# ssydasheng/GPflow-Slim

Hardware: AMD Instinct MI355X
Metric: GPR log-marginal-likelihood evals/sec + predict_f latency, fp64, N=32768 D=8 (higher is better)
Workload: dtype f64; 1 GPU; RBF(ARD) GPR log-marginal-likelihood, N=32768 D=8 R=1 fp64, X resident in HBM; n=32768, d=8, n_new=1024, parallelism=1 GPU (fused single-GPU path)

## Files before the change

### gpflow-slim_amd/csrc/blocked.hpp

```cpp
#pragma once
#include <cstdint>

#ifndef GPS_TILE
#define GPS_TILE 128
#endif

struct GemmBatch { int64_t batch = 1; int64_t a_rs = 0, a_cs = 0, a_cm = 0, b_rs = 0, b_cs = 0, b_cm = 0, c_rs = 0, c_cs = 0, c_cm = 0; };

template <class Ops>
struct Blocked {
  Ops& ops;
  explicit Blocked(Ops& o) : ops(o) {}
  typedef int64_t i64;

  static i64 split(i64 n) { return ((n / GPS_TILE) / 2) * GPS_TILE; }
  static i64 split_solve(i64 n) {
    const i64 P = 4 * GPS_TILE;
    if (n <= P) return split(n);
    const i64 h = ((n / P) / 2) * P;
    return h > P ? h : P;
  }

  struct Deferred { double* B; i64 ldb, dm, dn; bool issued; };

// ... 220 lines not shown
  int lauum_rec(const double* Y, i64 ldy, i64 n, double* Kv, i64 ldk) {
    if (n <= 0) return 0;
    if (n == GPS_TILE) return ops.gemm(1, 1, n, n, n, Y, ldy, Y, ldy, Kv, ldk);
    const i64 n1 = split(n), n2 = n - n1;
    int rc = lauum_rec(Y, ldy, n1, Kv, ldk);
    if (rc) return rc;
    const double* Y12 = Y + n1;
    const double* Y22 = Y + n1 * ldy + n1;
    rc = ops.gemm(2, 1, n1, n1, n2, Y12, ldy, Y12, ldy, Kv, ldk);
    if (rc) return rc;
    rc = ops.gemm(1,  2, n2, n1, n2, Y22, ldy, Y12, ldy, Kv + n1 * ldk, ldk);
    if (rc) return rc;
    return lauum_rec(Y22, ldy, n2, Kv + n1 * ldk + n1, ldk);
  }

  int trsv_rec(const double* L, i64 ldl, i64 n, i64 blk0, double* y, i64 ldy, i64 r) {
    if (n <= 0 || r <= 0) return 0;
    if (n == GPS_TILE) return ops.trsv_base(blk0, y, ldy, r, L, ldl);
    const i64 n1 = split(n), n2 = n - n1;
    int rc = trsv_rec(L, ldl, n1, blk0, y, ldy, r);
    if (rc) return rc;
    rc = ops.gemv_sub(L + n1 * ldl, ldl, n2, n1, y, y + n1, ldy, r);
    if (rc) return rc;
    return trsv_rec(L + n1 * ldl + n1, ldl, n2, blk0 + n1 / GPS_TILE, y + n1, ldy, r);
  }

  int wide_inverse(const double* L, i64 ldl, i64 nf, i64 wb, const double* linv, const double* linvT, double* W, double* Wt, double* Tm) {
    if (nf <= 0) return 0;
    const i64 T = GPS_TILE, ldt = wb / 2;
    int rc = ops.blocks_to_diag(linv, W, nf / T, wb);
// ... 28 lines not shown
```

### gpflow-slim_amd/csrc/gemm_f64.hip

```cpp
#include "gps_common.hpp"

typedef double v4d __attribute__((ext_vector_type(4)));
typedef double v2d __attribute__((ext_vector_type(2)));

#define BK_MIN 16
#ifndef STRIP
#define STRIP 8
#endif

struct GemmArgs {
  const double* A; const double* B; double* C;
  i64 lda, ldb, ldc;
  int Tm, Tn;
  int K;
  int ntiles;
  int triA;
  int batch, tpb;
  int pair;
  i64 a_rs, a_cs, b_rs, b_cs, c_rs, c_cs, a_cm, b_cm, c_cm;
  int cb_tiles;
  i64 cb_stride;
  int cb_cpack = 0;
  int nfull, nsplit;
  double* ws;
// ... 164 lines not shown
  }
  const i64 nbatch = (bt && bt->batch > 1) ? bt->batch : 1;
  const bool half_rows = (M % 128 == 64) && !lower && triA != 1 && triA != 2 && nbatch == 1;
  if ((M % 128 && !half_rows) || N % 128 || K % BK_MIN || (lower && M < N))
    return gps_fail(h, GPS_ERR_ARG, "gemm_nt: M,N must be multiples of 128 and K of 16 (lower: M >= N)");
  if ((lda & 1) || (ldb & 1) || ((uintptr_t)A & 15) || ((uintptr_t)B & 15))
    return gps_fail(h, GPS_ERR_ARG, "gemm_nt: operands must be 16-byte aligned with even leading dimension");
  const bool rowpanel = (C == A);
  if (rowpanel && (N != 128 || lower || triA || nbatch > 1))
    return gps_fail(h, GPS_ERR_ARG, "gemm_nt: in-place form needs N == 128 (no batch, no triangular operand)");
  GemmArgs g;
  g.A = A; g.B = B; g.C = C; g.lda = lda; g.ldb = ldb; g.ldc = ldc; g.K = (int)K; g.triA = triA;
  g.batch = (int)nbatch; g.tpb = 0;
  g.a_rs = g.a_cs = g.b_rs = g.b_cs = g.c_rs = g.c_cs = g.a_cm = g.b_cm = g.c_cm = 0;
  if (nbatch > 1) {
    if (lower) return gps_fail(h, GPS_ERR_ARG, "gemm_nt: no batched lower-triangle form");
    g.a_rs = bt->a_rs; g.a_cs = bt->a_cs; g.a_cm = bt->a_cm; g.b_rs = bt->b_rs; g.b_cs = bt->b_cs; g.b_cm = bt->b_cm;
    g.c_rs = bt->c_rs; g.c_cs = bt->c_cs; g.c_cm = bt->c_cm;
    if ((g.a_cs & 1) || (g.b_cs & 1) || (g.a_cm & 1) || (g.b_cm & 1)) return gps_fail(h, GPS_ERR_ARG, "gemm_nt: batch column steps must be even");
  }
  g.stamps = h->gemm_stamps;
  g.sig_ptr = h->next_sig_ptr; g.sig_val = h->next_sig_val; h->next_sig_ptr = nullptr;
  g.cb_tiles = 0; g.cb_stride = 0;
  const double t128 = (double)nbatch * (lower ? 0.5 * (double)(N / 128) * (double)(N / 128 + 1) + (double)((M - N) / 128) * (double)(N / 128)
                                             : ((double)M / 128.0) * (double)(N / 128));
  const double flops = triA == 3 ? (double)nbatch * 128.0 * 128.0 * ((double)M / 128.0) * (double)(N / 128) * (double)(N + 128)
                     : triA      ? (double)nbatch * 128.0 * 128.0 * (double)(N / 128) * (double)(M / 128) * (double)(M + 128)
                                 : 2.0 * t128 * 128.0 * 128.0 * (double)K;
  const double bytes = t128 * (((op == 0 || op == 2) ? 2.0 : 1.0) * 128.0 * 128.0 * 8.0) +
                       8.0 * (double)K * (double)(M + N);
  LaunchScope ls(h, KC_GEMM, flops, bytes);
// ... 10 lines not shown
    if (bm == 64) return launch_cfg<64, 128, 2>(h, op, 0, g, M, N);
    if (bm == 32) return launch_cfg<32, 128, 1>(h, op, 0, g, M, N);
    return launch_cfg<16, 128, 1>(h, op, 0, g, M, N);
  }
  int tb = 32;
  if (force) tb = force < 32 ? 32 : force;
  else if (t128 >= target && !half_rows) tb = 128;
  else if (4.0 * t128 >= target) tb = 64;
  if (half_rows && tb > 64) tb = 64;
  if (tb == 128) return launch_cfg<128, 128, 2>(h, op, lower, g, M, N);
  if (tb == 64) return launch_cfg<64, 64, 2>(h, op, lower, g, M, N);
  return launch_cfg<32, 32, 2>(h, op, lower, g, M, N);
}

int gps_launch_gemm_nt_dual(gps_handle_t h, i64 M, i64 N, i64 K, const double* A, i64 lda, const double* B, i64 ldb,
                            double* C, i64 ldc, double* C2, i64 ldc2, int op2) {
  if (M <= 0 || N <= 0 || K <= 0) return GPS_OK;
  if (M % 128 || N % 128 || K % BK_MIN || !C || !C2 || (op2 != 0 && op2 != 2))
    return gps_fail(h, GPS_ERR_ARG, "gemm_nt_dual: M,N must be multiples of 128 and K of 16, two targets, op2 0 or 2");
  if ((lda & 1) || (ldb & 1) || ((uintptr_t)A & 15) || ((uintptr_t)B & 15))
    return gps_fail(h, GPS_ERR_ARG, "gemm_nt_dual: operands must be 16-byte aligned with even leading dimension");
  if (C == A || C2 == A || C == C2) return gps_fail(h, GPS_ERR_ARG, "gemm_nt_dual: no in-place form");
  if ((M / 128) * (N / 128) > 0x7fffffff) return gps_fail(h, GPS_ERR_ARG, "gemm_nt: too many tiles");
  GemmArgs g;
  g.A = A; g.B = B; g.C = C; g.lda = lda; g.ldb = ldb; g.ldc = ldc; g.K = (int)K; g.triA = 0;
  g.batch = 1; g.pair = 0;
  g.a_rs = g.a_cs = g.b_rs = g.b_cs = g.c_rs = g.c_cs = g.a_cm = g.b_cm = g.c_cm = 0;
  g.cb_tiles = 0; g.cb_stride = 0;
  g.Tm = (int)(M / 128); g.Tn = (int)(N / 128);
  g.ntiles = g.Tm * g.Tn; g.tpb = g.ntiles;
  g.nfull = g.ntiles; g.nsplit = 1; g.ws = nullptr; g.cnt = nullptr;
  g.stamps = nullptr;
  g.sig_ptr = h->next_sig_ptr; g.sig_val = h->next_sig_val; h->next_sig_ptr = nullptr;
  g.C2 = C2; g.ldc2 = ldc2; g.op2 = op2;
  const double t128 = (double)g.ntiles;
  LaunchScope ls(h, KC_GEMM, 2.0 * t128 * 128.0 * 128.0 * (double)K, t128 * 4.0 * 128.0 * 128.0 * 8.0 + 8.0 * (double)K * (double)(M + N));
  ls.tag[0] = M; ls.tag[1] = N; ls.tag[2] = K; ls.tag[3] = 50 + op2;
  const size_t lds = (size_t)(2 * (128 + 128) * (16 + 2)) * sizeof(double);
  int rc = gps_dyn_lds(h, reinterpret_cast<const void*>(&gemm_nt_f64_kernel<128, 128, 2, false, 0, 2, 16, true>), (int)lds);
  if (rc) return rc;
  hipLaunchKernelGGL((gemm_nt_f64_kernel<128, 128, 2, false, 0, 2, 16, true>), dim3(g.ntiles), dim3(256), lds, h->stream, g);
  GPS_HIP(h, hipGetLastError());
  return GPS_OK;
}

int gps_launch_gemm_nt_cyclic(gps_handle_t h, i64 M, i64 nblocks, i64 nb, i64 stride, i64 K, const double* A, i64 lda,
                              double* C, i64 ldc, int c_packed) {
  if (M <= 0 || nblocks <= 0) return GPS_OK;
  if (M % 128 || nb % 128 || stride % 128 || K % BK_MIN || stride < nb || (nblocks - 1) * stride + nb > M)
    return gps_fail(h, GPS_ERR_ARG, "gemm_nt_cyclic: sizes must be multiples of 128 and the blocks must lie inside the panel");
  GemmArgs g;
  g.A = A; g.B = A; g.C = C; g.lda = lda; g.ldb = lda; g.ldc = ldc; g.K = (int)K; g.triA = 0;
  g.batch = 1; g.tpb = 0; g.pair = 0; g.a_rs = g.a_cs = g.b_rs = g.b_cs = g.c_rs = g.c_cs = g.a_cm = g.b_cm = g.c_cm = 0;
// ... 15 lines not shown
```

### gpflow-slim_amd/csrc/gps_common.hpp

```cpp
#pragma once
#include <hip/hip_runtime.h>
#include <cmath>
#include <cstdint>
#include <cstdio>
#include <cstring>
#include <cstdlib>
#include <string>
#include <vector>
#include "../../include/gpflowslim_hip.h"
#include "blocked.hpp"

#define GPS_TILE 128
#define GPS_WB 2048
#define GPS_WIDE_MAX_ROWS 8192

typedef int64_t i64;

static inline i64 gps_pad(i64 n) { return ((n + GPS_TILE - 1) / GPS_TILE) * GPS_TILE; }

struct DevBuf;
typedef std::vector<DevBuf*> DevBufList;
struct DevBuf {
  enum Class { WORK, PERSISTENT };
  void*  p = nullptr;
// ... 194 lines not shown
    int on = 1;
    int fault_inject = 0;
    long long fallbacks = 0;
    int consec = 0;
    int cooldown = 0;
    bool defer = false;
    bool pending = false;
    bool valid = false;
    double slog = 0.0, ssq = 0.0;
    bool linvT_stale = false;
  } small;
  DevBuf dGemmWs{bufs}, dGemmCnt{bufs};
  int gemm_strassen_min = 2048;
  static constexpr int strassen_min_builtin = 2048, strassen_lower_min_builtin = 4096;
  int gemm_strassen_lower_min = strassen_lower_min_builtin;
  DevBuf dStrS{bufs}, dStrT{bufs};
  int gemm_strassen_presum_min = 1024;
  double gemm_strassen_presum_max_bytes = 0.0;
  long long strassen_presum_fallbacks = 0;
  DevBuf dStrS5{bufs}, dStrT5{bufs};
  struct RffFactor { bool have = false; unsigned long long gen = 0; i64 F = 0, r = 0; int kind = -1, d = 0; bool refine = false; } rff;
  DevBuf dGemvWs{bufs}, dGemvCnt{bufs};
  struct KgprSolve { bool have = false; unsigned long long gen = 0; i64 m = 0, n = 0; } kgpr;
  int kron_cg_check_every = 8;
  int psi_sum_chunk = 0;
  DevBuf dPsiParts{bufs};
  DevBuf dPsiWork{bufs};
  struct GpmcState { bool have = false; unsigned long long gen = 0; i64 n = 0, k = 0; } gpmc;
};

// ... 98 lines not shown
  GPS_HIP(h, hipFuncSetAttribute(fn, hipFuncAttributeMaxDynamicSharedMemorySize, bytes));
  h->dyn_lds_done.push_back(fn);
  return GPS_OK;
}

int gps_launch_gemm_nt(gps_handle_t h, int op, int lower, i64 M, i64 N, i64 K,
                       const double* A, i64 lda, const double* B, i64 ldb,
                       double* C, i64 ldc);
struct GemmBatch;
int gps_launch_gemm_nt_ex(gps_handle_t h, int op, int lower, int tri, i64 M, i64 N, i64 K,
                          const double* A, i64 lda, const double* B, i64 ldb,
                          double* C, i64 ldc, const GemmBatch* bt);
int gps_launch_gemm_nt_cyclic(gps_handle_t h, i64 M, i64 nblocks, i64 nb, i64 stride, i64 K, const double* A, i64 lda,
                              double* C, i64 ldc, int c_packed = 0);
int gps_launch_gemm_nt_dual(gps_handle_t h, i64 M, i64 N, i64 K, const double* A, i64 lda, const double* B, i64 ldb,
                            double* C, i64 ldc, double* C2, i64 ldc2, int op2);
int gps_launch_block_sum(gps_handle_t h, double* D, i64 ldd, const double* X, i64 ldx, const double* Y, i64 ldy, i64 rows, i64 cols,
                         int sign);
int gps_launch_strassen_sums(gps_handle_t h, int side, const double* X, i64 ldx, i64 rows, i64 cols, double* out, i64 ostride);
int gps_launch_potrf_base(gps_handle_t h, double* A, i64 lda, double* Linv_blk,
                          double* LinvT_blk, int* d_info, i64 row0, int factor,
                          long long* d_stamps = nullptr);
int gps_launch_trsm_leaf_refine(gps_handle_t h, double* B, i64 ldb, i64 m, const double* W, const double* D, i64 ldd,
                                int upper);
int gps_launch_trsv_leaf_refine(gps_handle_t h, const double* Wt, const double* D, i64 ldd, double* y, i64 ldy, i64 r,
                                int upper);
static inline bool gps_gpr_needs_refine(const gps_handle_s* h, double noise_var, double kdiag, i64 n) {
  if (h->leaf_refine >= 0) return h->leaf_refine > 0;
  return !((double)n * kdiag + noise_var <= h->leaf_refine_cond * noise_var);
}

// ... 206 lines not shown
```

### gpflow-slim_amd/csrc/gps_gpr.hip

```cpp
#include "gps_ops.hpp"

static int gpr_lml_finish(gps_handle_t h, i64 r, double* lml);
extern "C" int gps_kmat(gps_handle_t h, const gps_kern_node_t* prog, int n_nodes, const double* X,
                        int64_t n, const double* X2, int64_t m, int64_t d_all, double diag_add,
                        double* K_out) {
  if (!h || !X || !K_out || n < 0 || d_all <= 0) return gps_fail(h, GPS_ERR_ARG, "gps_kmat: bad argument");
  GPS_HIP(h, hipSetDevice(h->device));
  const bool sym = (X2 == nullptr);
  if (sym) m = n;
  if (n == 0 || m == 0) return GPS_OK;
  const i64 prow = ((n + 63) / 64) * 64;
  const i64 pcol = sym ? prow : ((m + 63) / 64) * 64;
  GPS_HIP(h, h->dXnew.ensure((size_t)n * d_all * 8));
  GPS_HIP(h, hipMemcpyAsync(h->dXnew.p, X, (size_t)n * d_all * 8, hipMemcpyHostToDevice, h->stream));
  const double* dX2 = nullptr;
  if (!sym) {
    GPS_HIP(h, h->dTmp3.ensure((size_t)m * d_all * 8));
    GPS_HIP(h, hipMemcpyAsync(h->dTmp3.p, X2, (size_t)m * d_all * 8, hipMemcpyHostToDevice, h->stream));
    dX2 = h->dTmp3.d();
  }
  GPS_HIP(h, h->dTmp.ensure((size_t)prow * pcol * 8));
  int rc = gps_launch_kmat(h, prog, n_nodes, h->dXnew.d(), n, dX2, m, d_all, diag_add, h->dTmp.d(), pcol,
                           prow, pcol,  0,  0);
  if (rc) return rc;
// ... 321 lines not shown
static int gpr_kinv_small(gps_handle_t h, i64 r, double* d_abort, double* d_AT) {
  int rc = gpr_kinv_buffers(h, r);
  if (rc) return rc;
  return gps_launch_small_inverse(h, h->dK.d(), h->npad, h->dLinv.d(), h->dAlpha.d(), r, h->dY.d(), h->dKinv.d(), h->dA.d(), d_abort, d_AT, h->n);
}
static int gpr_kinv_blocked(gps_handle_t h, i64 r) {
  const i64 np = h->npad;
  int rc = gpr_kinv_buffers(h, r);
  if (!rc) rc = gpr_ensure_linvT(h);
  if (rc) return rc;
  HipOps ops = factor_ops(h, h->dLinv.d(), np, (int*)h->dInfo.p);
  Blocked<HipOps> bl(ops);
  GPS_HIP(h, hipMemcpyAsync(h->dA.p, h->dAlpha.p, (size_t)r * np * 8, hipMemcpyDeviceToDevice, h->stream));
  rc = trsv_backward(h, ops, h->dK.d(), np, np, h->dA.d(), np, r);
  if (rc) return rc;
  rc = bl.inv_t_rec(h->dK.d(), np, np, 0, h->dY.d(), np);
  if (rc) return rc;
  return bl.lauum_rec(h->dY.d(), np, np, h->dKinv.d(), np);
}
static int gpr_grad_readback(gps_handle_t h, const gps_kern_node_t* prog, int n_nodes, i64 r, double* grad_slots, double* grad_noise,
                             double* kinv_resid) {
  const i64 n = h->n, np = h->npad;
  int rc = gps_launch_grad(h, prog, n_nodes, h->dX.d(), n, h->d_all, np, h->dKinv.d(), np, h->dA.d(), np, r, nullptr, grad_slots, grad_noise);
  if (rc || !kinv_resid) return rc;
  GPS_HIP(h, h->dTmp2.ensure((size_t)n * r * 8));
  rc = gps_launch_transpose(h, h->dA.d(), np, r, n, h->dTmp2.d(), r);
  if (rc) return rc;
  GPS_HIP(h, hipMemcpyAsync(kinv_resid, h->dTmp2.p, (size_t)n * r * 8, hipMemcpyDeviceToHost, h->stream));
  return GPS_OK;
}
// ... 185 lines not shown
```

### gpflow-slim_amd/csrc/gps_handle.hip

```cpp
#include "gps_ops.hpp"

extern "C" int gps_create(int device_id, gps_handle_t* out) {
  if (!out) return GPS_ERR_ARG;
  *out = nullptr;
  int count = 0;
  if (hipGetDeviceCount(&count) != hipSuccess || count <= 0) return GPS_ERR_HIP;
  if (device_id < 0 || device_id >= count) return GPS_ERR_ARG;
  gps_handle_t h = new gps_handle_s();
  h->device = device_id;
  if (hipSetDevice(device_id) != hipSuccess || hipGetDeviceProperties(&h->prop, device_id) != hipSuccess) {
    delete h;
    return GPS_ERR_HIP;
  }
  if (hipStreamCreateWithFlags(&h->stream, hipStreamNonBlocking) != hipSuccess) { delete h; return GPS_ERR_HIP; }
  for (int i = 0; i < 8; ++i) {
    if (hipEventCreate(&h->ev[i]) != hipSuccess) { delete h; return GPS_ERR_HIP; }
  }
  if (const char* v = getenv("GPS_GEMM_PAIR")) h->gemm_pair = atoi(v);
  if (const char* la = getenv("GPS_LOOKAHEAD")) h->potrf_lookahead = atoi(la);
  if (h->dInfo.ensure(64) != hipSuccess || h->dScal.ensure(4096) != hipSuccess) { delete h; return GPS_ERR_HIP; }
  *out = h;
  return GPS_OK;
}

// ... 98 lines not shown
  }
  return gps_fail(h, GPS_ERR_ARG, "unknown kernel class");
}
extern "C" int gps_last_stage_ms(gps_handle_t h, double* out5) {
  if (!h || !out5) return GPS_ERR_ARG;
  for (int i = 0; i < 5; ++i) out5[i] = h->stage_ms[i];
  return GPS_OK;
}

static int set_strassen_tuning(gps_handle_t h, const char* sub, double value) {
  const bool lower_min = strcmp(sub, "lower_min") == 0;
  if (lower_min || strcmp(sub, "presum_min") == 0) {
    if (value < 0 || value > 1e9 || value != (double)((i64)value) || (i64)value % 128)
      return gps_fail(h, GPS_ERR_ARG, std::string("gemm_strassen_") + sub + ": 0 or a multiple of 128");
    (lower_min ? h->gemm_strassen_lower_min : h->gemm_strassen_presum_min) = (int)value;
    return GPS_OK;
  }
  if (strcmp(sub, "presum_max_bytes") == 0) {
    if (!(value >= 0)) return gps_fail(h, GPS_ERR_ARG, "gemm_strassen_presum_max_bytes: 0 (no cap) or a number of bytes");
    h->gemm_strassen_presum_max_bytes = value;
    return GPS_OK;
  }
  return gps_fail(h, GPS_ERR_ARG, "unknown option");
}

extern "C" int gps_set_option(gps_handle_t h, const char* key, double value) {
  if (!h || !key) return GPS_ERR_ARG;
  if (strcmp(key, "gemm_force_tile") == 0) { h->gemm_force_tb = (int)value; return GPS_OK; }
  if (strcmp(key, "gemm_tail_split") == 0) { h->gemm_tail_split = (int)value; return GPS_OK; }
  if (strcmp(key, "gemm_strassen_min") == 0) {
// ... 37 lines not shown
  return gps_run_mfma_diag(h, waves_per_simd, tflops, layout_ok);
}

extern "C" int gps_diag_gemm_nt(gps_handle_t h, int op, int lower, int64_t m, int64_t n, int64_t k,
                                const double* A, const double* B, double* C) {
  if (!h || !A || !B || !C) return GPS_ERR_ARG;
  GPS_HIP(h, hipSetDevice(h->device));
  const size_t ab = (size_t)m * k * 8, bb = (size_t)n * k * 8, cb = (size_t)m * n * 8;
  GPS_HIP(h, h->dTmp.ensure(ab)); GPS_HIP(h, h->dTmp2.ensure(bb)); GPS_HIP(h, h->dTmp3.ensure(cb));
  GPS_HIP(h, hipMemcpyAsync(h->dTmp.p, A, ab, hipMemcpyHostToDevice, h->stream));
  GPS_HIP(h, hipMemcpyAsync(h->dTmp2.p, B, bb, hipMemcpyHostToDevice, h->stream));
  GPS_HIP(h, hipMemcpyAsync(h->dTmp3.p, C, cb, hipMemcpyHostToDevice, h->stream));
  h->refine_now = false;
  HipOps ops{h, nullptr, nullptr, nullptr};
  int rc = lower >= 3 ? gps_launch_gemm_nt_ex(h, op, 0, lower - 1, m, n, k, h->dTmp.d(), k, h->dTmp2.d(), k, h->dTmp3.d(), n, nullptr)
         : lower == 2 ? gps_launch_gemm_nt(h, op, lower, m, n, k, h->dTmp.d(), k, h->dTmp2.d(), k, h->dTmp3.d(), n)
                      : ops.gemm(op, lower, m, n, k, h->dTmp.d(), k, h->dTmp2.d(), k, h->dTmp3.d(), n);
  if (rc) return rc;
  GPS_HIP(h, hipMemcpyAsync(C, h->dTmp3.p, cb, hipMemcpyDeviceToHost, h->stream));
  GPS_HIP(h, hipStreamSynchronize(h->stream));
  return GPS_OK;
}

extern "C" int gps_diag_gemm_nt_batched(gps_handle_t h, int op, int tri, int64_t batch, int64_t m, int64_t n, int64_t k,
                                        const double* A, const double* B, double* C) {
  if (!h || !A || !B || !C || batch < 1) return GPS_ERR_ARG;
  GPS_HIP(h, hipSetDevice(h->device));
  const size_t ab = (size_t)batch * m * k * 8, bb = (size_t)batch * n * k * 8, cb = (size_t)batch * m * n * 8;
  GPS_HIP(h, h->dTmp.ensure(ab)); GPS_HIP(h, h->dTmp2.ensure(bb)); GPS_HIP(h, h->dTmp3.ensure(cb));
  GPS_HIP(h, hipMemcpyAsync(h->dTmp.p, A, ab, hipMemcpyHostToDevice, h->stream));
  GPS_HIP(h, hipMemcpyAsync(h->dTmp2.p, B, bb, hipMemcpyHostToDevice, h->stream));
// ... 250 lines not shown
```

### gpflow-slim_amd/csrc/gps_ops.hpp

```cpp
#pragma once
#include "gps_common.hpp"
#include "blocked.hpp"
#include "strassen.hpp"
#include "dist_schedule.hpp"
#include <climits>
#include <cmath>
#include <algorithm>

size_t gps_tri_skinny_part_doubles(i64 n, i64 r);
int gps_launch_tri_skinny(gps_handle_t h, int trans, const double* L, i64 ldl, i64 n, const double* Bt, i64 ldb, i64 r, double* Ft,
                          i64 ldf, double* part);
int gps_launch_chol_seed(gps_handle_t h, const double* Ut, i64 ldu, const double* Vt, i64 ldv, i64 r, i64 n, double* P, i64 ldp, i64 np,
                         int accumulate = 0);
size_t gps_skinny_xt_part_doubles(i64 rows, i64 mp, i64 r);
int gps_launch_skinny_xt(gps_handle_t h, const double* X, i64 ld, i64 rows, i64 mp, const double* Et, i64 lde, i64 r, double* Gt, i64 ldg,
                         int accumulate, double* part);

static int planes_upload(gps_handle_t h, const double* src, i64 n, i64 k, double* stage, double* planes, i64 np) {
  GPS_HIP(h, hipMemcpyAsync(stage, src, (size_t)n * k * 8, hipMemcpyHostToDevice, h->stream));
  GPS_HIP(h, hipMemsetAsync(planes, 0, (size_t)k * np * 8, h->stream));
  return gps_launch_transpose(h, stage, k, n, k, planes, np);
}
static int planes_download(gps_handle_t h, const double* planes, i64 np, i64 n, i64 k, double* stage, double* dst) {
  int rc = gps_launch_transpose(h, planes, np, k, n, stage, k);
// ... 48 lines not shown
  int trsm_leaf512(i64 blk, int transposed, double* B, i64 ldb, i64 m, const double* D, i64 ldd) {
    if (h->refine_now) h->leaves_plain += 4;
    const double* W = (transposed ? linvT : linv) + blk * GPS_TILE * GPS_TILE;
    return gps_launch_trsm_panel(h, B, ldb, m, D, ldd, W, transposed);
  }
  bool on_main_stream() const {
    if (saved_stream || saved_stream_d) return false;
    if (h->side_stream && h->stream == h->side_stream) return false;
    if (h->def_stream && h->stream == h->def_stream) return false;
    if (h->dist.bulk_set && h->stream == h->dist.bulk_stream) return false;
    return true;
  }
  int gemm(int op, int lower, i64 M, i64 N, i64 K, const double* A, i64 lda, const double* B,
           i64 ldb, double* C, i64 ldc) {
    const i64 smin = h->gemm_strassen_min;
    if (smin > 0 && op == 0 && !h->refine_now && C != A && on_main_stream()) {
      if (lower == 0 && strassen_shape_ok(M, N, K, smin)) {
        const size_t sb = (size_t)(M / 2) * (size_t)(K / 2) * 8, tb = (size_t)(N / 2) * (size_t)(K / 2) * 8;
        if (strassen_shape_ok(M, N, K, h->gemm_strassen_presum_min) && presum_buffers(5 * sb, 5 * tb)) {
          const int rc = strassen_nt_presummed(*this, M, N, K, A, lda, B, ldb, C, ldc, h->dStrS5.d(), h->dStrT5.d());
          return rc < 0 ? gps_fail(h, GPS_ERR_ARG, "strassen_nt_presummed: bad shape") : rc;
        }
        GPS_HIP(h, h->dStrS.ensure(sb));
        GPS_HIP(h, h->dStrT.ensure(tb));
        const int rc = strassen_nt(*this, M, N, K, A, lda, B, ldb, C, ldc, h->dStrS.d(), h->dStrT.d());
        return rc < 0 ? gps_fail(h, GPS_ERR_ARG, "strassen_nt: bad shape") : rc;
      }
      int rc = 0;
      if (lower == 1 && strassen_lower_split(*this, M, N, K, A, lda, B, ldb, C, ldc, h->gemm_strassen_lower_min, &rc)) return rc;
    }
    return gemm_plain(op, lower, M, N, K, A, lda, B, ldb, C, ldc);
  }
  bool presum_buffers(size_t s_bytes, size_t t_bytes) {
    const double cap = h->gemm_strassen_presum_max_bytes;
    bool ok = !(cap > 0.0 && (double)s_bytes + (double)t_bytes > cap);
    if (ok && (s_bytes > h->dStrS5.cap || t_bytes > h->dStrT5.cap)) {
      size_t need = 0, back = 0, free_b = 0, total_b = 0;
      if (s_bytes > h->dStrS5.cap) { need += s_bytes + ((size_t)1 << 20); back += h->dStrS5.cap; }
      if (t_bytes > h->dStrT5.cap) { need += t_bytes + ((size_t)1 << 20); back += h->dStrT5.cap; }
      ok = hipMemGetInfo(&free_b, &total_b) == hipSuccess && need <= free_b + back;
      if (ok) {
        ok = h->dStrS5.ensure(s_bytes) == hipSuccess && h->dStrT5.ensure(t_bytes) == hipSuccess;
        if (!ok) { h->dStrS5.release(); h->dStrT5.release(); }
      }
      if (!ok) (void)hipGetLastError();
    }
    if (!ok) h->strassen_presum_fallbacks++;
    return ok;
  }
  int sums(int side, const double* X, i64 ldx, i64 r, i64 c, double* out, i64 out_stride) {
    return gps_launch_strassen_sums(h, side, X, ldx, r, c, out, out_stride);
  }
  int add(double* D, i64 ldd, const double* X, i64 ldx, const double* Y, i64 ldy, i64 rows, i64 cols, int sign) {
    return gps_launch_block_sum(h, D, ldd, X, ldx, Y, ldy, rows, cols, sign);
  }
  int gemm2(i64 M, i64 N, i64 K, const double* A, i64 lda, const double* B, i64 ldb, double* C, i64 ldc, double* C2, i64 ldc2, int op2) {
    if (!C2) return gps_launch_gemm_nt(h, 0, 0, M, N, K, A, lda, B, ldb, C, ldc);
    return gps_launch_gemm_nt_dual(h, M, N, K, A, lda, B, ldb, C, ldc, C2, ldc2, op2);
  }
  int gemm_plain(int op, int lower, i64 M, i64 N, i64 K, const double* A, i64 lda, const double* B,
                 i64 ldb, double* C, i64 ldc) {
    if (h->follower_max_wgs > 0 && op == 0 && !lower && h->def_stream && h->stream == h->def_stream && M >= 128 && N > 128) {
      const i64 rows = (M + 127) / 128;
      const i64 w = std::max<i64>(1, h->follower_max_wgs / rows) * 128;
      if (w < N) {
        for (i64 u = 0; u < N; u += w) {
          const int rc = gps_launch_gemm_nt(h, op, lower, M, std::min(w, N - u), K, A, lda, B + u * ldb, ldb, C + u, ldc);
          if (rc) return rc;
        }
        return GPS_OK;
      }
    }
    return gps_launch_gemm_nt(h, op, lower, M, N, K, A, lda, B, ldb, C, ldc);
  }
  int gemm_ex(int op, int tri, i64 M, i64 N, i64 K, const double* A, i64 lda, const double* B, i64 ldb, double* C, i64 ldc, const GemmBatch* bt) {
    return gps_launch_gemm_nt_ex(h, op, 0, tri, M, N, K, A, lda, B, ldb, C, ldc, bt);
  }
  int blocks_to_diag(const double* src, double* dst, i64 nblk, i64 wb) { return gps_launch_blocks_to_diag(h, src, dst, nblk, wb); }
  int trsv_base(i64 blk, double* y, i64 ldy, i64 r, const double* D, i64 ldd) {
    if (!linvT) return gps_fail(h, GPS_ERR_STATE, "trsv needs the transposed block inverses");
    if (h->refine_now) return gps_launch_trsv_leaf_refine(h, linvT + blk * GPS_TILE * GPS_TILE, D, ldd, y, ldy, r, 0);
    return gps_launch_trsv_base(h, linvT + blk * GPS_TILE * GPS_TILE, y, ldy, r);
  }
  int gemv_sub(const double* L21, i64 ldl, i64 n2, i64 n1, const double* y1, double* y2, i64 ldy,
               i64 r) {
    return gps_launch_gemv_sub(h, L21, ldl, n2, n1, y1, y2, ldy, r);
  }
  int trsv_t_base(i64 blk, double* y, i64 ldy, i64 r, const double* D, i64 ldd) {
    if (h->refine_now) return gps_launch_trsv_leaf_refine(h, linv + blk * GPS_TILE * GPS_TILE, D, ldd, y, ldy, r, 1);
    return gps_launch_trsv_base(h, linv + blk * GPS_TILE * GPS_TILE, y, ldy, r);
  }
// ... 296 lines not shown
```

### gpflow-slim_amd/csrc/strassen.hpp

```cpp
#pragma once
#include <cstdint>

template <class Ops>
int strassen_nt(Ops& ops, int64_t M, int64_t N, int64_t K, const double* A, int64_t lda, const double* B, int64_t ldb, double* C,
                int64_t ldc, double* S, double* T) {
  typedef int64_t i64;
  if (M <= 0 || N <= 0 || K <= 0) return 0;
  if (M % 256 || N % 256 || K % 256) return -1;
  const i64 m = M / 2, n = N / 2, k = K / 2;
  const double* A11 = A;            const double* A12 = A + k;
  const double* A21 = A + m * lda;  const double* A22 = A21 + k;
  const double* B11 = B;            const double* B12 = B + k;
  const double* B21 = B + n * ldb;  const double* B22 = B21 + k;
  double* C11 = C;            double* C12 = C + n;
  double* C21 = C + m * ldc;  double* C22 = C21 + n;
  int rc;
  if ((rc = ops.add(S, k, A11, lda, A22, lda, m, k, +1))) return rc;
  if ((rc = ops.add(T, k, B11, ldb, B22, ldb, n, k, +1))) return rc;
  if ((rc = ops.gemm2(m, n, k, S, k, T, k, C11, ldc, C22, ldc, 0))) return rc;
  if ((rc = ops.add(S, k, A21, lda, A22, lda, m, k, +1))) return rc;
  if ((rc = ops.gemm2(m, n, k, S, k, B11, ldb, C21, ldc, C22, ldc, 2))) return rc;
  if ((rc = ops.add(T, k, B21, ldb, B22, ldb, n, k, -1))) return rc;
  if ((rc = ops.gemm2(m, n, k, A11, lda, T, k, C12, ldc, C22, ldc, 0))) return rc;
  if ((rc = ops.add(T, k, B12, ldb, B11, ldb, n, k, -1))) return rc;
// ... 21 lines not shown
  double* C21 = C + m * ldc;  double* C22 = C21 + n;
  const double* S[5]; const double* T[5];
  for (int q = 0; q < 5; ++q) { S[q] = S5 + q * m * k; T[q] = T5 + q * n * k; }
  int rc;
  if ((rc = ops.sums(0, A, lda, m, k, S5, m * k))) return rc;
  if ((rc = ops.sums(1, B, ldb, n, k, T5, n * k))) return rc;
  if ((rc = ops.gemm2(m, n, k, S[0], k, T[0], k, C11, ldc, C22, ldc, 0))) return rc;
  if ((rc = ops.gemm2(m, n, k, S[1], k, B11, ldb, C21, ldc, C22, ldc, 2))) return rc;
  if ((rc = ops.gemm2(m, n, k, A11, lda, T[1], k, C12, ldc, C22, ldc, 0))) return rc;
  if ((rc = ops.gemm2(m, n, k, A22, lda, T[2], k, C11, ldc, C21, ldc, 0))) return rc;
  if ((rc = ops.gemm2(m, n, k, S[2], k, B22, ldb, C12, ldc, C11, ldc, 2))) return rc;
  if ((rc = ops.gemm2(m, n, k, S[3], k, T[3], k, C22, ldc, nullptr, 0, 0))) return rc;
  return ops.gemm2(m, n, k, S[4], k, T[4], k, C11, ldc, nullptr, 0, 0);
}

static inline bool strassen_shape_ok(int64_t M, int64_t N, int64_t K, int64_t min_quadrant) {
  if (min_quadrant <= 0 || M % 256 || N % 256 || K % 256) return false;
  return M / 2 >= min_quadrant && N / 2 >= min_quadrant && K / 2 >= min_quadrant;
}

template <class Ops>
bool strassen_lower_split(Ops& ops, int64_t M, int64_t N, int64_t K, const double* A, int64_t lda, const double* B, int64_t ldb,
                          double* C, int64_t ldc, int64_t min_quadrant, int* rc_out) {
  typedef int64_t i64;
  const i64 n = N / 2;
  if (min_quadrant <= 0 || M < N || N % 256 || n / 2 < min_quadrant || !strassen_shape_ok(n, n, K, min_quadrant)) return false;
  int rc = ops.gemm_plain(0, 1, n, n, K, A, lda, B, ldb, C, ldc);
  if (!rc) rc = ops.gemm(0, 0, n, n, K, A + n * lda, lda, B, ldb, C + n * ldc, ldc);
  if (!rc && M > N) rc = ops.gemm_plain(0, 0, M - N, n, K, A + N * lda, lda, B, ldb, C + N * ldc, ldc);
  if (!rc) rc = ops.gemm_plain(0, 1, M - n, n, K, A + n * lda, lda, B + n * ldb, ldb, C + n * ldc + n, ldc);
  *rc_out = rc;
  return true;
}
```

Measured before the change: 5.715 evals/s.

## Extend Strassen to accumulate/triangular GEMMs and batch small-level Kinv inversion

Routes the K-inverse path (triangular inverse followed by LAUUM) through a new wide-block scheme. The levels below a 2048 block width are done as batched GEMMs, including a new batched lower-triangle form, and the recursion above them reuses Strassen. Strassen now also covers subtract/accumulate GEMMs (op 2), lower-split accumulate and an upper-triangular split, backed by a dual-output kernel variant that accumulates. The aim is to cut launch count and flops in the O(n^3) inverse at N=32768. The cost is extra workspace, more fp64 rounding error from Strassen, and new code paths.

After: 5.702 evals/s. No clear change (-0.2%).

```diff
diff --git a/gpflow-slim_amd/csrc/blocked.hpp b/gpflow-slim_amd/csrc/blocked.hpp
--- a/gpflow-slim_amd/csrc/blocked.hpp
+++ b/gpflow-slim_amd/csrc/blocked.hpp
@@ -258,6 +258,79 @@
     return lauum_rec(Y22, ldy, n2, Kv + n1 * ldk + n1, ldk);
   }
 
+  static bool wide_ok(i64 n, i64 wb) {
+    if (wb < 2 * GPS_TILE || n < wb || n % wb) return false;
+    for (i64 b = GPS_TILE; b <= wb; b *= 2) if (b == wb) { const i64 q = n / wb; return (q & (q - 1)) == 0; }
+    return false;
+  }
+  int inv_t_wide(const double* L, i64 ldl, i64 n, i64 wb, const double* linv, const double* linvT, double* W, double* Tm, double* Y, i64 ldy) {
+    if (n <= 0) return 0;
+    if (!wide_ok(n, wb)) return inv_t_rec(L, ldl, n, 0, Y, ldy);
+    const i64 T = GPS_TILE, ldt = wb / 2;
+    int rc = ops.blocks_to_diag(linv, W, n / T, wb);
+    if (!rc) rc = ops.blocks_to_diag(linvT, Y, n / T, ldy);
+    for (i64 b = T; b < wb && !rc; b *= 2) {
+      GemmBatch bt;
+      bt.batch = n / (2 * b);
+      bt.a_rs = 2 * b; bt.a_cs = 2 * b; bt.a_cm = 0; bt.b_rs = 2 * b; bt.b_cs = 2 * b; bt.b_cm = 0; bt.c_rs = b; bt.c_cs = 0; bt.c_cm = 0;
+      rc = ops.gemm_ex( 1,  1, b, b, b, Y, ldy, L + b * ldl, ldl, Tm, ldt, &bt);
+      if (rc) break;
+      bt.a_rs = b; bt.a_cs = 0; bt.a_cm = 0; bt.b_rs = 2 * b; bt.b_cs = 2 * b; bt.b_cm = wb; bt.c_rs = 2 * b; bt.c_cs = 2 * b; bt.c_cm = 0;
+      rc = ops.gemm_ex( 3,  3, b, b, b, Tm, ldt, W + b * wb + b, wb, Y + b, ldy, &bt);
+      if (!rc && ops.fill_zeros())
+        for (i64 p = 0; p < bt.batch && !rc; ++p) rc = ops.zero_block(Y + (2 * b * p + b) * ldy + 2 * b * p, ldy, b, b);
+      if (rc || 2 * b >= wb) break;
+      bt.a_rs = 2 * b; bt.a_cs = 2 * b; bt.a_cm = wb; bt.b_rs = b; bt.b_cs = 0; bt.b_cm = 0; bt.c_rs = 2 * b; bt.c_cs = 2 * b; bt.c_cm = wb;
+      rc = ops.gemm_ex(3,  2, b, b, b, W + b * wb + b, wb, Tm, ldt, W + b * wb, wb, &bt);
+    }
+    return rc ? rc : inv_t_above(L, ldl, n, 0, wb, Y, ldy);
+  }
+  int inv_t_above(const double* L, i64 ldl, i64 n, i64 blk0, i64 wb, double* Y, i64 ldy) {
+    if (n <= wb) return 0;
+    const i64 n1 = n / 2, n2 = n - n1;
+    int rc = inv_t_above(L, ldl, n1, blk0, wb, Y, ldy);
+    if (rc) return rc;
+    rc = inv_t_above(L + n1 * ldl + n1, ldl, n2, blk0 + n1 / GPS_TILE, wb, Y + n1 * ldy + n1, ldy);
+    if (rc) return rc;
+    double* Y12 = Y + n1;
+    if (ops.fill_zeros()) {
+      rc = ops.zero_block(Y + n1 * ldy, ldy, n2, n1);
+      if (rc) return rc;
+    }
+    rc = ops.gemm( 3,  2, n1, n2, n1, Y, ldy, L + n1 * ldl, ldl, Y12, ldy);
+    if (rc) return rc;
+    return trsm_rec(L + n1 * ldl + n1, ldl, n2, blk0 + n1 / GPS_TILE, Y12, ldy, n1);
+  }
+  int lauum_wide(const double* Y, i64 ldy, i64 n, i64 wb, double* Kv, i64 ldk) {
+    if (n <= 0) return 0;
+    if (!wide_ok(n, wb)) return lauum_rec(Y, ldy, n, Kv, ldk);
+    const i64 T = GPS_TILE;
+    GemmBatch bt;
+    bt.batch = n / T;
+    bt.a_rs = bt.a_cs = bt.b_rs = bt.b_cs = bt.c_rs = bt.c_cs = T;
+    int rc = ops.gemm_ex( 1, 0, T, T, T, Y, ldy, Y, ldy, Kv, ldk, &bt);
+    for (i64 b = T; b < wb && !rc; b *= 2) {
+      bt.batch = n / (2 * b);
+      bt.a_rs = bt.a_cs = bt.b_rs = bt.b_cs = bt.c_rs = bt.c_cs = 2 * b;
+      rc = ops.gemm_lower_batched( 2, b, b, b, Y + b, ldy, Y + b, ldy, Kv, ldk, &bt);
+      if (!rc) rc = ops.gemm_ex(1,  1, b, b, b, Y + b * ldy + b, ldy, Y + b, ldy, Kv + b * ldk, ldk, &bt);
+    }
+    return rc ? rc : lauum_above(Y, ldy, n, wb, Kv, ldk);
+  }
+  int lauum_above(const double* Y, i64 ldy, i64 n, i64 wb, double* Kv, i64 ldk) {
+    if (n <= wb) return 0;
+    const i64 n1 = n / 2, n2 = n - n1;
+    int rc = lauum_above(Y, ldy, n1, wb, Kv, ldk);
+    if (rc) return rc;
+    const double* Y12 = Y + n1;
+    const double* Y22 = Y + n1 * ldy + n1;
+    rc = ops.gemm(2, 1, n1, n1, n2, Y12, ldy, Y12, ldy, Kv, ldk);
+    if (rc) return rc;
+    rc = ops.gemm(1,  2, n2, n1, n2, Y22, ldy, Y12, ldy, Kv + n1 * ldk, ldk);
+    if (rc) return rc;
+    return lauum_above(Y22, ldy, n2, wb, Kv + n1 * ldk + n1, ldk);
+  }
+
   int trsv_rec(const double* L, i64 ldl, i64 n, i64 blk0, double* y, i64 ldy, i64 r) {
     if (n <= 0 || r <= 0) return 0;
     if (n == GPS_TILE) return ops.trsv_base(blk0, y, ldy, r, L, ldl);
diff --git a/gpflow-slim_amd/csrc/gemm_f64.hip b/gpflow-slim_amd/csrc/gemm_f64.hip
--- a/gpflow-slim_amd/csrc/gemm_f64.hip
+++ b/gpflow-slim_amd/csrc/gemm_f64.hip
@@ -202,7 +202,7 @@
   g.batch = (int)nbatch; g.tpb = 0;
   g.a_rs = g.a_cs = g.b_rs = g.b_cs = g.c_rs = g.c_cs = g.a_cm = g.b_cm = g.c_cm = 0;
   if (nbatch > 1) {
-    if (lower) return gps_fail(h, GPS_ERR_ARG, "gemm_nt: no batched lower-triangle form");
+    if (lower && M != N) return gps_fail(h, GPS_ERR_ARG, "gemm_nt: a batched lower-triangle form must be square");
     g.a_rs = bt->a_rs; g.a_cs = bt->a_cs; g.a_cm = bt->a_cm; g.b_rs = bt->b_rs; g.b_cs = bt->b_cs; g.b_cm = bt->b_cm;
     g.c_rs = bt->c_rs; g.c_cs = bt->c_cs; g.c_cm = bt->c_cm;
     if ((g.a_cs & 1) || (g.b_cs & 1) || (g.a_cm & 1) || (g.b_cm & 1)) return gps_fail(h, GPS_ERR_ARG, "gemm_nt: batch column steps must be even");
@@ -243,9 +243,9 @@
 }
 
 int gps_launch_gemm_nt_dual(gps_handle_t h, i64 M, i64 N, i64 K, const double* A, i64 lda, const double* B, i64 ldb,
-                            double* C, i64 ldc, double* C2, i64 ldc2, int op2) {
+                            double* C, i64 ldc, double* C2, i64 ldc2, int op2, int op) {
   if (M <= 0 || N <= 0 || K <= 0) return GPS_OK;
-  if (M % 128 || N % 128 || K % BK_MIN || !C || !C2 || (op2 != 0 && op2 != 2))
+  if (M % 128 || N % 128 || K % BK_MIN || !C || !C2 || (op2 != 0 && op2 != 2) || (op != 0 && op != 2))
     return gps_fail(h, GPS_ERR_ARG, "gemm_nt_dual: M,N must be multiples of 128 and K of 16, two targets, op2 0 or 2");
   if ((lda & 1) || (ldb & 1) || ((uintptr_t)A & 15) || ((uintptr_t)B & 15))
     return gps_fail(h, GPS_ERR_ARG, "gemm_nt_dual: operands must be 16-byte aligned with even leading dimension");
@@ -264,8 +264,15 @@
   g.C2 = C2; g.ldc2 = ldc2; g.op2 = op2;
   const double t128 = (double)g.ntiles;
   LaunchScope ls(h, KC_GEMM, 2.0 * t128 * 128.0 * 128.0 * (double)K, t128 * 4.0 * 128.0 * 128.0 * 8.0 + 8.0 * (double)K * (double)(M + N));
-  ls.tag[0] = M; ls.tag[1] = N; ls.tag[2] = K; ls.tag[3] = 50 + op2;
+  ls.tag[0] = M; ls.tag[1] = N; ls.tag[2] = K; ls.tag[3] = 50 + op2 + 2 * op;
   const size_t lds = (size_t)(2 * (128 + 128) * (16 + 2)) * sizeof(double);
+  if (op == 2) {
+    int rc = gps_dyn_lds(h, reinterpret_cast<const void*>(&gemm_nt_f64_kernel<128, 128, 2, false, 2, 2, 16, true>), (int)lds);
+    if (rc) return rc;
+    hipLaunchKernelGGL((gemm_nt_f64_kernel<128, 128, 2, false, 2, 2, 16, true>), dim3(g.ntiles), dim3(256), lds, h->stream, g);
+    GPS_HIP(h, hipGetLastError());
+    return GPS_OK;
+  }
   int rc = gps_dyn_lds(h, reinterpret_cast<const void*>(&gemm_nt_f64_kernel<128, 128, 2, false, 0, 2, 16, true>), (int)lds);
   if (rc) return rc;
   hipLaunchKernelGGL((gemm_nt_f64_kernel<128, 128, 2, false, 0, 2, 16, true>), dim3(g.ntiles), dim3(256), lds, h->stream, g);
diff --git a/gpflow-slim_amd/csrc/gps_common.hpp b/gpflow-slim_amd/csrc/gps_common.hpp
--- a/gpflow-slim_amd/csrc/gps_common.hpp
+++ b/gpflow-slim_amd/csrc/gps_common.hpp
@@ -232,6 +232,9 @@
   int gemm_strassen_min = 2048;
   static constexpr int strassen_min_builtin = 2048, strassen_lower_min_builtin = 4096;
   int gemm_strassen_lower_min = strassen_lower_min_builtin;
+  int gemm_strassen_kinv = 1;
+  int gemm_strassen_kinv_wide = 2048;
+  DevBuf dKinvW{bufs};
   DevBuf dStrS{bufs}, dStrT{bufs};
   int gemm_strassen_presum_min = 1024;
   double gemm_strassen_presum_max_bytes = 0.0;
@@ -360,7 +363,7 @@
 int gps_launch_gemm_nt_cyclic(gps_handle_t h, i64 M, i64 nblocks, i64 nb, i64 stride, i64 K, const double* A, i64 lda,
                               double* C, i64 ldc, int c_packed = 0);
 int gps_launch_gemm_nt_dual(gps_handle_t h, i64 M, i64 N, i64 K, const double* A, i64 lda, const double* B, i64 ldb,
-                            double* C, i64 ldc, double* C2, i64 ldc2, int op2);
+                            double* C, i64 ldc, double* C2, i64 ldc2, int op2, int op = 0);
 int gps_launch_block_sum(gps_handle_t h, double* D, i64 ldd, const double* X, i64 ldx, const double* Y, i64 ldy, i64 rows, i64 cols,
                          int sign);
 int gps_launch_strassen_sums(gps_handle_t h, int side, const double* X, i64 ldx, i64 rows, i64 cols, double* out, i64 ostride);
diff --git a/gpflow-slim_amd/csrc/gps_gpr.hip b/gpflow-slim_amd/csrc/gps_gpr.hip
--- a/gpflow-slim_amd/csrc/gps_gpr.hip
+++ b/gpflow-slim_amd/csrc/gps_gpr.hip
@@ -359,6 +359,14 @@
   GPS_HIP(h, hipMemcpyAsync(h->dA.p, h->dAlpha.p, (size_t)r * np * 8, hipMemcpyDeviceToDevice, h->stream));
   rc = trsv_backward(h, ops, h->dK.d(), np, np, h->dA.d(), np, r);
   if (rc) return rc;
+  const i64 wb = (h->refine_now || !ops.on_main_stream()) ? 0 : h->gemm_strassen_kinv_wide;
+  if (Blocked<HipOps>::wide_ok(np, wb)) {
+    GPS_HIP(h, h->dKinvW.ensure((size_t)np * wb * 8));
+    GPS_HIP(h, h->dBigT.ensure((size_t)(np / 2) * (wb / 2) * 8));
+    rc = bl.inv_t_wide(h->dK.d(), np, np, wb, ops.linv, ops.linvT, h->dKinvW.d(), h->dBigT.d(), h->dY.d(), np);
+    if (rc) return rc;
+    return bl.lauum_wide(h->dY.d(), np, np, wb, h->dKinv.d(), np);
+  }
   rc = bl.inv_t_rec(h->dK.d(), np, np, 0, h->dY.d(), np);
   if (rc) return rc;
   return bl.lauum_rec(h->dY.d(), np, np, h->dKinv.d(), np);
diff --git a/gpflow-slim_amd/csrc/gps_handle.hip b/gpflow-slim_amd/csrc/gps_handle.hip
--- a/gpflow-slim_amd/csrc/gps_handle.hip
+++ b/gpflow-slim_amd/csrc/gps_handle.hip
@@ -136,6 +136,14 @@
     if (value < 0 || value > 1e9 || value != (double)((i64)value) || (i64)value % 128)
       return gps_fail(h, GPS_ERR_ARG, std::string("gemm_strassen_") + sub + ": 0 or a multiple of 128");
     (lower_min ? h->gemm_strassen_lower_min : h->gemm_strassen_presum_min) = (int)value;
+    return GPS_OK;
+  }
+  if (strcmp(sub, "kinv") == 0) { h->gemm_strassen_kinv = value != 0.0; return GPS_OK; }
+  if (strcmp(sub, "kinv_wide") == 0) {
+    const i64 v = (i64)value;
+    if (value < 0 || value > 1e9 || value != (double)v || (v && (v < 256 || v % 128 || ((v / 128) & (v / 128 - 1)))))
+      return gps_fail(h, GPS_ERR_ARG, "gemm_strassen_kinv_wide: 0 or 128 times a power of two, at least 256");
+    h->gemm_strassen_kinv_wide = (int)v;
     return GPS_OK;
   }
   if (strcmp(sub, "presum_max_bytes") == 0) {
@@ -203,7 +211,6 @@
   h->refine_now = false;
   HipOps ops{h, nullptr, nullptr, nullptr};
   int rc = lower >= 3 ? gps_launch_gemm_nt_ex(h, op, 0, lower - 1, m, n, k, h->dTmp.d(), k, h->dTmp2.d(), k, h->dTmp3.d(), n, nullptr)
-         : lower == 2 ? gps_launch_gemm_nt(h, op, lower, m, n, k, h->dTmp.d(), k, h->dTmp2.d(), k, h->dTmp3.d(), n)
                       : ops.gemm(op, lower, m, n, k, h->dTmp.d(), k, h->dTmp2.d(), k, h->dTmp3.d(), n);
   if (rc) return rc;
   GPS_HIP(h, hipMemcpyAsync(C, h->dTmp3.p, cb, hipMemcpyDeviceToHost, h->stream));
diff --git a/gpflow-slim_amd/csrc/gps_ops.hpp b/gpflow-slim_amd/csrc/gps_ops.hpp
--- a/gpflow-slim_amd/csrc/gps_ops.hpp
+++ b/gpflow-slim_amd/csrc/gps_ops.hpp
@@ -86,20 +86,24 @@
   int gemm(int op, int lower, i64 M, i64 N, i64 K, const double* A, i64 lda, const double* B,
            i64 ldb, double* C, i64 ldc) {
     const i64 smin = h->gemm_strassen_min;
-    if (smin > 0 && op == 0 && !h->refine_now && C != A && on_main_stream()) {
-      if (lower == 0 && strassen_shape_ok(M, N, K, smin)) {
+    if (smin > 0 && (op == 0 || h->gemm_strassen_kinv) && !h->refine_now && C != A && on_main_stream()) {
+      int rc = 0;
+      if ((op == 0 || op == 2) && lower == 0 && strassen_shape_ok(M, N, K, smin)) {
         const size_t sb = (size_t)(M / 2) * (size_t)(K / 2) * 8, tb = (size_t)(N / 2) * (size_t)(K / 2) * 8;
         if (strassen_shape_ok(M, N, K, h->gemm_strassen_presum_min) && presum_buffers(5 * sb, 5 * tb)) {
-          const int rc = strassen_nt_presummed(*this, M, N, K, A, lda, B, ldb, C, ldc, h->dStrS5.d(), h->dStrT5.d());
+          rc = op == 0 ? strassen_nt_presummed(*this, M, N, K, A, lda, B, ldb, C, ldc, h->dStrS5.d(), h->dStrT5.d())
+                       : strassen_nt_signed_presummed(*this, M, N, K, A, lda, B, ldb, C, ldc, h->dStrS5.d(), h->dStrT5.d());
           return rc < 0 ? gps_fail(h, GPS_ERR_ARG, "strassen_nt_presummed: bad shape") : rc;
         }
         GPS_HIP(h, h->dStrS.ensure(sb));
         GPS_HIP(h, h->dStrT.ensure(tb));
-        const int rc = strassen_nt(*this, M, N, K, A, lda, B, ldb, C, ldc, h->dStrS.d(), h->dStrT.d());
+        rc = op == 0 ? strassen_nt(*this, M, N, K, A, lda, B, ldb, C, ldc, h->dStrS.d(), h->dStrT.d())
+                     : strassen_nt_signed(*this, M, N, K, A, lda, B, ldb, C, ldc, h->dStrS.d(), h->dStrT.d());
         return rc < 0 ? gps_fail(h, GPS_ERR_ARG, "strassen_nt: bad shape") : rc;
       }
-      int rc = 0;
-      if (lower == 1 && strassen_lower_split(*this, M, N, K, A, lda, B, ldb, C, ldc, h->gemm_strassen_lower_min, &rc)) return rc;
+      if ((op == 0 || op == 2) && lower == 1 &&
+          strassen_lower_split(*this, M, N, K, A, lda, B, ldb, C, ldc, h->gemm_strassen_lower_min, &rc, op)) return rc;
+      if (lower == 2 && M == K && strassen_upper_split(*this, op, M, N, A, lda, B, ldb, C, ldc, smin, &rc)) return rc;
     }
     return gemm_plain(op, lower, M, N, K, A, lda, B, ldb, C, ldc);
   }
@@ -130,6 +134,10 @@
     if (!C2) return gps_launch_gemm_nt(h, 0, 0, M, N, K, A, lda, B, ldb, C, ldc);
     return gps_launch_gemm_nt_dual(h, M, N, K, A, lda, B, ldb, C, ldc, C2, ldc2, op2);
   }
+  int gemm2_add(i64 M, i64 N, i64 K, const double* A, i64 lda, const double* B, i64 ldb, double* C, i64 ldc, double* C2, i64 ldc2, int op2) {
+    if (!C2) return gps_launch_gemm_nt(h, 2, 0, M, N, K, A, lda, B, ldb, C, ldc);
+    return gps_launch_gemm_nt_dual(h, M, N, K, A, lda, B, ldb, C, ldc, C2, ldc2, op2,  2);
+  }
   int gemm_plain(int op, int lower, i64 M, i64 N, i64 K, const double* A, i64 lda, const double* B,
                  i64 ldb, double* C, i64 ldc) {
     if (h->follower_max_wgs > 0 && op == 0 && !lower && h->def_stream && h->stream == h->def_stream && M >= 128 && N > 128) {
@@ -147,6 +155,9 @@
   }
   int gemm_ex(int op, int tri, i64 M, i64 N, i64 K, const double* A, i64 lda, const double* B, i64 ldb, double* C, i64 ldc, const GemmBatch* bt) {
     return gps_launch_gemm_nt_ex(h, op, 0, tri, M, N, K, A, lda, B, ldb, C, ldc, bt);
+  }
+  int gemm_lower_batched(int op, i64 M, i64 N, i64 K, const double* A, i64 lda, const double* B, i64 ldb, double* C, i64 ldc, const GemmBatch* bt) {
+    return gps_launch_gemm_nt_ex(h, op, 1, 0, M, N, K, A, lda, B, ldb, C, ldc, bt);
   }
   int blocks_to_diag(const double* src, double* dst, i64 nblk, i64 wb) { return gps_launch_blocks_to_diag(h, src, dst, nblk, wb); }
   int trsv_base(i64 blk, double* y, i64 ldy, i64 r, const double* D, i64 ldd) {
diff --git a/gpflow-slim_amd/csrc/strassen.hpp b/gpflow-slim_amd/csrc/strassen.hpp
--- a/gpflow-slim_amd/csrc/strassen.hpp
+++ b/gpflow-slim_amd/csrc/strassen.hpp
@@ -59,6 +59,64 @@
   return ops.gemm2(m, n, k, S[4], k, T[4], k, C11, ldc, nullptr, 0, 0);
 }
 
+template <class Ops>
+int strassen_nt_signed(Ops& ops, int64_t M, int64_t N, int64_t K, const double* A, int64_t lda, const double* B, int64_t ldb,
+                       double* C, int64_t ldc, double* S, double* T) {
+  typedef int64_t i64;
+  if (M <= 0 || N <= 0 || K <= 0) return 0;
+  if (M % 256 || N % 256 || K % 256) return -1;
+  const i64 m = M / 2, n = N / 2, k = K / 2;
+  const double* A11 = A;            const double* A12 = A + k;
+  const double* A21 = A + m * lda;  const double* A22 = A21 + k;
+  const double* B11 = B;            const double* B12 = B + k;
+  const double* B21 = B + n * ldb;  const double* B22 = B21 + k;
+  double* C11 = C;            double* C12 = C + n;
+  double* C21 = C + m * ldc;  double* C22 = C21 + n;
+  int rc;
+  if ((rc = ops.add(S, k, A11, lda, A22, lda, m, k, +1))) return rc;
+  if ((rc = ops.add(T, k, B11, ldb, B22, ldb, n, k, +1))) return rc;
+  if ((rc = ops.gemm2_add(m, n, k, S, k, T, k, C11, ldc, C22, ldc, 2))) return rc;
+  if ((rc = ops.add(S, k, A21, lda, A22, lda, m, k, +1))) return rc;
+  if ((rc = ops.gemm2_add(m, n, k, S, k, B11, ldb, C21, ldc, C22, ldc, 0))) return rc;
+  if ((rc = ops.add(T, k, B21, ldb, B22, ldb, n, k, -1))) return rc;
+  if ((rc = ops.gemm2_add(m, n, k, A11, lda, T, k, C12, ldc, C22, ldc, 2))) return rc;
+  if ((rc = ops.add(T, k, B12, ldb, B11, ldb, n, k, -1))) return rc;
+  if ((rc = ops.gemm2_add(m, n, k, A22, lda, T, k, C11, ldc, C21, ldc, 2))) return rc;
+  if ((rc = ops.add(S, k, A11, lda, A12, lda, m, k, +1))) return rc;
+  if ((rc = ops.gemm2_add(m, n, k, S, k, B22, ldb, C12, ldc, C11, ldc, 0))) return rc;
+  if ((rc = ops.add(S, k, A21, lda, A11, lda, m, k, -1))) return rc;
+  if ((rc = ops.add(T, k, B11, ldb, B21, ldb, n, k, +1))) return rc;
+  if ((rc = ops.gemm2_add(m, n, k, S, k, T, k, C22, ldc, nullptr, 0, 0))) return rc;
+  if ((rc = ops.add(S, k, A12, lda, A22, lda, m, k, -1))) return rc;
+  if ((rc = ops.add(T, k, B12, ldb, B22, ldb, n, k, +1))) return rc;
+  return ops.gemm2_add(m, n, k, S, k, T, k, C11, ldc, nullptr, 0, 0);
+}
+
+template <class Ops>
+int strassen_nt_signed_presummed(Ops& ops, int64_t M, int64_t N, int64_t K, const double* A, int64_t lda, const double* B,
+                                 int64_t ldb, double* C, int64_t ldc, double* S5, double* T5) {
+  typedef int64_t i64;
+  if (M <= 0 || N <= 0 || K <= 0) return 0;
+  if (M % 256 || N % 256 || K % 256) return -1;
+  const i64 m = M / 2, n = N / 2, k = K / 2;
+  const double* A11 = A;            const double* A22 = A + m * lda + k;
+  const double* B11 = B;            const double* B22 = B + n * ldb + k;
+  double* C11 = C;            double* C12 = C + n;
+  double* C21 = C + m * ldc;  double* C22 = C21 + n;
+  const double* S[5]; const double* T[5];
+  for (int q = 0; q < 5; ++q) { S[q] = S5 + q * m * k; T[q] = T5 + q * n * k; }
+  int rc;
+  if ((rc = ops.sums(0, A, lda, m, k, S5, m * k))) return rc;
+  if ((rc = ops.sums(1, B, ldb, n, k, T5, n * k))) return rc;
+  if ((rc = ops.gemm2_add(m, n, k, S[0], k, T[0], k, C11, ldc, C22, ldc, 2))) return rc;
+  if ((rc = ops.gemm2_add(m, n, k, S[1], k, B11, ldb, C21, ldc, C22, ldc, 0))) return rc;
+  if ((rc = ops.gemm2_add(m, n, k, A11, lda, T[1], k, C12, ldc, C22, ldc, 2))) return rc;
+  if ((rc = ops.gemm2_add(m, n, k, A22, lda, T[2], k, C11, ldc, C21, ldc, 2))) return rc;
+  if ((rc = ops.gemm2_add(m, n, k, S[2], k, B22, ldb, C12, ldc, C11, ldc, 0))) return rc;
+  if ((rc = ops.gemm2_add(m, n, k, S[3], k, T[3], k, C22, ldc, nullptr, 0, 0))) return rc;
+  return ops.gemm2_add(m, n, k, S[4], k, T[4], k, C11, ldc, nullptr, 0, 0);
+}
+
 static inline bool strassen_shape_ok(int64_t M, int64_t N, int64_t K, int64_t min_quadrant) {
   if (min_quadrant <= 0 || M % 256 || N % 256 || K % 256) return false;
   return M / 2 >= min_quadrant && N / 2 >= min_quadrant && K / 2 >= min_quadrant;
@@ -66,14 +124,27 @@
 
 template <class Ops>
 bool strassen_lower_split(Ops& ops, int64_t M, int64_t N, int64_t K, const double* A, int64_t lda, const double* B, int64_t ldb,
-                          double* C, int64_t ldc, int64_t min_quadrant, int* rc_out) {
+                          double* C, int64_t ldc, int64_t min_quadrant, int* rc_out, int op = 0) {
   typedef int64_t i64;
   const i64 n = N / 2;
   if (min_quadrant <= 0 || M < N || N % 256 || n / 2 < min_quadrant || !strassen_shape_ok(n, n, K, min_quadrant)) return false;
-  int rc = ops.gemm_plain(0, 1, n, n, K, A, lda, B, ldb, C, ldc);
-  if (!rc) rc = ops.gemm(0, 0, n, n, K, A + n * lda, lda, B, ldb, C + n * ldc, ldc);
-  if (!rc && M > N) rc = ops.gemm_plain(0, 0, M - N, n, K, A + N * lda, lda, B, ldb, C + N * ldc, ldc);
-  if (!rc) rc = ops.gemm_plain(0, 1, M - n, n, K, A + n * lda, lda, B + n * ldb, ldb, C + n * ldc + n, ldc);
+  int rc = ops.gemm_plain(op, 1, n, n, K, A, lda, B, ldb, C, ldc);
+  if (!rc) rc = ops.gemm(op, 0, n, n, K, A + n * lda, lda, B, ldb, C + n * ldc, ldc);
+  if (!rc && M > N) rc = ops.gemm_plain(op, 0, M - N, n, K, A + N * lda, lda, B, ldb, C + N * ldc, ldc);
+  if (!rc) rc = ops.gemm_plain(op, 1, M - n, n, K, A + n * lda, lda, B + n * ldb, ldb, C + n * ldc + n, ldc);
   *rc_out = rc;
   return true;
 }
+
+template <class Ops>
+bool strassen_upper_split(Ops& ops, int op, int64_t M, int64_t N, const double* A, int64_t lda, const double* B, int64_t ldb, double* C,
+                          int64_t ldc, int64_t min_quadrant, int* rc_out) {
+  typedef int64_t i64;
+  const i64 m = M / 2;
+  if ((op != 1 && op != 3) || !strassen_shape_ok(m, N, m, min_quadrant)) return false;
+  int rc = ops.gemm_plain(op, 2, m, N, m, A, lda, B, ldb, C, ldc);
+  if (!rc) rc = ops.gemm(op == 3 ? 0 : 2, 0, m, N, m, A + m, lda, B + m, ldb, C, ldc);
+  if (!rc) rc = ops.gemm_plain(op, 2, m, N, m, A + m * lda + m, lda, B + m, ldb, C + m * ldc, ldc);
+  *rc_out = rc;
+  return true;
+}
```
